# goldbricklemon/uplift-upsample-3dhpe

Hardware: AMD Instinct MI355X
Metric: pose-sequences/sec (higher is better)
Workload: dtype f16x3 (f32 operands split into f16 hi/lo, 3 MFMA passes, f32 accumulate); 1 GPU; config/h36m_351.json forward, N=71 tokens (receptive field 351), J=17, batch 128/GPU, s_in=5, seeded Keras-default weights; global_batch=128, parallelism=batch-sharded x1, hipgraph=True, concurrent_half_batches=False, batches_in_flight=8

## Files before the change

### uplift-upsample-3dhpe_amd/csrc/uu3d_api.hip

```cpp
#include <hip/hip_runtime.h>

#include <algorithm>
#include <cmath>
#include <cstdio>
#include <cstdlib>
#include <cstring>
#include <functional>
#include <map>
#include <mutex>
#include <string>
#include <vector>

#include "../../include/uu3d.h"
#include "uu3d_switches.h"
#include "uu3d_gemm.h"
#include "uu3d_gemm_h3.h"
#include "uu3d_gemm_panel.h"
#include "uu3d_gemm_panel8.h"
#include "uu3d_gemm_wt.h"
#include "uu3d_mlp_fused.h"
#include "uu3d_tchain16.h"
#include "uu3d_attn.h"
#include "uu3d_attn_h3.h"
#include "uu3d_spatial.h"
#include "uu3d_spatial_h3.h"
#include "uu3d_spatial_p16.h"
#include "uu3d_misc.h"
#include "uu3d_metrics.h"
#include "uu3d_tracks.h"
#include "uu3d_stream.h"
#include "uu3d_train.h"
#include "uu3d_bwd.h"
#include "uu3d_launch.h"
#include "uu3d_train_kernels.h"

using namespace uu3d;

namespace {

constexpr int kJ = 17, kDS = 32, kHS = 64, kHeads = 8, kDH = 48;
using SLY2 = SpatialBlockLayoutV2<kDS, kHS>;
constexpr int kFR = 3;
#ifndef UU3D_SPATIAL_MT
#define UU3D_SPATIAL_MT 1
#endif
constexpr int kP16FR = 7, kP16PW = 1;
constexpr int kSpatialMT = UU3D_SPATIAL_MT;

std::string g_create_error;

inline int round_up(int v, int m) { return (v + m - 1) / m * m; }
inline size_t align_up(size_t v, size_t a) { return (v + a - 1) / a * a; }

struct WeightRec {
    std::string name;
    std::vector<int64_t> dims;
    int64_t numel = 0;
    std::vector<float> host;
    bool set = false;
};

struct BlockDev {
    const float *ln1_g, *ln1_b, *wqkv_t, *bqkv, *wp_t, *bp, *ln2_g, *ln2_b, *w1_t, *b1, *w2_t, *b2;
    const float* pe;
    size_t wqkv_pf = 0, w1_pf = 0;
    size_t w2_mf = 0;
    size_t wp_pf = 0;
};

struct ProfRec {
    std::string name, kernel;
    double flops, bytes;
    hipEvent_t e0, e1;
};

}

struct uu3d_train_state;
struct uu3d_model {
    uu3d_config cfg;
    uu3d_train_state* ts = nullptr;
    int device = 0;
    std::vector<WeightRec> weights;
    std::map<std::string, int> index;
    std::vector<int> L;
    Switches sw;
    bool committed = false;
    bool generic = false;
    float* gparams = nullptr;
    float* arena = nullptr;
    size_t arena_floats = 0;
    bool throughput = false;
    struct TcLaunch { int flags; size_t w_off ; size_t p_off ; };
    std::vector<TcLaunch> tchain;
    int num_cus = 256;
    std::recursive_mutex train_mu;
    bool in_commit = false;
    int* d_range = nullptr;
    _Float16* harena = nullptr;
    size_t harena_halfs = 0;
    std::map<size_t, std::pair<size_t, size_t>> hplanes;
    std::map<size_t, size_t> panel_off, mlpf_off;
    SpatialParams sp{};
    size_t sp_frag_off = 0;
// ... 570 lines not shown
```

### uplift-upsample-3dhpe_amd/csrc/uu3d_forward.inc

```

namespace {
struct Workspace {
    float *S, *X, *QKV, *O, *Hb, *XA, *XB, *slab, *mslab;
    unsigned char* tc_scratch;
    int* frame_list;
    float2* stats;
    size_t slab_floats;
    size_t bytes;
};
Workspace carve(const uu3d_model* m, int B, char* base) {
    const uu3d_config& c = m->cfg;
    const size_t rows = (size_t)B * c.num_frames;
    const size_t rows_s = (size_t)B * (c.num_strided > 1 ? std::max(m->L[1], 1) : 1);
    size_t off = 0;
    auto take = [&](size_t n) { size_t o = off; off = align_up(off + n, 256); return o; };
    Workspace w{};
    const size_t oS = take(rows * c.num_keypoints * c.d_spatial * 4);
    const size_t oX = take(rows * c.d_temporal * 4);
    const size_t oQ = take((rows + 128) * 3 * c.d_temporal * 4);
    const size_t oO = take((rows + 32) * c.d_temporal * 4);
    const size_t oH = take((rows + 32) * c.h_temporal * 4);
    const size_t oA = take(rows * c.d_temporal * 4);
    const size_t oB = take(rows_s * c.d_temporal * 4);
    const size_t oT = take(rows * sizeof(float2));
// ... 38 lines not shown
    hipStream_t stream;
    float* slab = nullptr;
    size_t slab_floats = 0;
    bool throughput = false;
    int precision = UU3D_PREC_F16X3;
    int status = UU3D_OK;
    bool few_splits = false;

    void begin(const char* name, const char* kernel, double flops, double bytes) {
        if (!m->profiling) return;
        if (m->prof_used == m->prof.size()) {
            ProfRec r;
            if (hipEventCreate(&r.e0) != hipSuccess || hipEventCreate(&r.e1) != hipSuccess) { status = UU3D_ERR_HIP; return; }
            m->prof.push_back(r);
        }
        ProfRec& r = m->prof[m->prof_used];
        r.name = name; r.kernel = kernel; r.flops = flops; r.bytes = bytes;
        (void)hipEventRecord(r.e0, stream);
    }
    void end() {
        if (m->profiling && m->prof_used < m->prof.size()) { (void)hipEventRecord(m->prof[m->prof_used].e1, stream); ++m->prof_used; }
        hipError_t e = hipGetLastError();
        if (e != hipSuccess && status == UU3D_OK) { status = UU3D_ERR_HIP; m->err = std::string("kernel launch failed: ") + hipGetErrorString(e); }
    }

    template <int BM, int BN, class AL, class EP>
    void gemm_tile(const AL& al, const float* Bt, int M, int N, int Kp, int slices, int kt_per_split, const EP& ep) {
        auto kern = gemm_f32_kernel<BM, BN, AL, EP>;
        constexpr size_t lds = gemm_lds_bytes(BM, BN);
        allow_lds<gemm_f32_kernel<BM, BN, AL, EP>>(lds);
        const int mt = (M + BM - 1) / BM, nt = (N + BN - 1) / BN;
        const int grid = round_up(mt, 8) * nt;
        hipLaunchKernelGGL(kern, dim3(grid, slices), dim3(256), lds, stream, al, Bt, M, N, Kp, mt, nt, kt_per_split, ep);
    }

    template <int TM, int TN, class AL, class EP>
    void gemm_h3_tile(const AL& al, const _Float16* Bh, const _Float16* Bl, int M, int N, int Kp, int slices, int kt_per_split, const EP& ep) {
        auto kern = gemm_h3_kernel<TM, TN, AL, EP>;
        auto kern_deep = gemm_h3_kernel<TM, TN, AL, EP, 1>;
        constexpr size_t lds = gemm_h3_lds_bytes(64 * TM, 64 * TN);
        allow_lds<gemm_h3_kernel<TM, TN, AL, EP>>(lds); allow_lds<gemm_h3_kernel<TM, TN, AL, EP, 1>>(lds);
        const int mt = (M + 64 * TM - 1) / (64 * TM), nt = (N + 64 * TN - 1) / (64 * TN);
        const int grid = round_up(mt, 8) * nt;
        if (gemm_h3_deep(grid * slices)) hipLaunchKernelGGL(kern_deep, dim3(grid, slices), dim3(256), lds, stream, al, Bh, Bl, M, N, Kp, mt, nt, kt_per_split, ep);
        else hipLaunchKernelGGL(kern, dim3(grid, slices), dim3(256), lds, stream, al, Bh, Bl, M, N, Kp, mt, nt, kt_per_split, ep);
    }

    template <int TM, int TN, class GL, class EP>
    void gemm_h3g_tile(const GL& gl, const _Float16* Bh, const _Float16* Bl, int M, int N, int Kp, int slices, int kt_per_split, const EP& ep) {
        auto kern = gemm_h3g_kernel<TM, TN, GL, EP>;
        constexpr size_t lds = gemm_h3g_lds_bytes(64 * TM, 64 * TN);
        allow_lds<gemm_h3g_kernel<TM, TN, GL, EP>>(lds);
        const int mt = (M + 64 * TM - 1) / (64 * TM), nt = (N + 64 * TN - 1) / (64 * TN);
        const int grid = round_up(mt, 8) * nt;
        hipLaunchKernelGGL(kern, dim3(grid, slices), dim3(256), lds, stream, gl, Bh, Bl, M, N, Kp, mt, nt, kt_per_split, ep);
    }

    int splitk_target() const {
        return (throughput && few_splits) ? process_switches().thr_splitk_target : 768;
    }
    template <class GL, class EP>
    void gemm_g(const char* name, const GL& gl, const float* Bt, int M, int N, int K, const EP& ep, double extra_bytes = 0) {
        const int KT = K / 32;
        const int tiles = ((M + 63) / 64) * ((N + 63) / 64);
        const auto [slices, kps] = splitk_rule(M, N, KT, splitk_target(), slab_floats, true);
        const int ldslab = round_up(N, 4);
        begin(name, "gemm_h3", 2.0 * M * (double)N * K, 4.0 * ((double)M * K + (double)N * K + (double)M * N) + extra_bytes);
        const auto it = m->hplanes.find((size_t)(Bt - m->arena));
        if ((K % 32) != 0 || it == m->hplanes.end()) { status = UU3D_ERR_INVALID_ARGUMENT; m->err = "gemm_g: operand without f16 planes or K % 32 != 0"; end(); return; }
        const _Float16* Bh = m->harena + it->second.first; const _Float16* Bl = m->harena + it->second.second;
        if (slices == 1) {
            if (N % 128 == 0 && tiles >= 256) gemm_h3g_tile<1, 2>(gl, Bh, Bl, M, N, K, 1, KT, ep);
            else gemm_h3g_tile<1, 1>(gl, Bh, Bl, M, N, K, 1, KT, ep);
        } else {
            EpSlab es{slab, ldslab, (size_t)M * ldslab};
            if (N % 128 == 0 && tiles >= 200) gemm_h3g_tile<1, 2>(gl, Bh, Bl, M, N, K, slices, kps, es);
            else gemm_h3g_tile<1, 1>(gl, Bh, Bl, M, N, K, slices, kps, es);
            hipLaunchKernelGGL(splitk_reduce_kernel<EP>, dim3((M * N + 255) / 256), dim3(256), 0, stream,
                               slab, slices, (size_t)M * ldslab, M, N, ldslab, ep);
        }
        end();
    }

    static int panel_splits(int M, int N) {
        const int mt = (M + 127) / 128, chunks = N / 32;
        int best = 0; double best_cost = 1e30;
        for (int S = 1; S <= chunks; ++S) {
            if (chunks % S != 0 || chunks / S > PANEL_COLV_FLOATS / 32) continue;
            const int per_xcd = (mt * S + 7) / 8;
            const double cost = (double)((per_xcd + 31) / 32) * (2.5 + (double)chunks / S);
            if (cost < best_cost) { best_cost = cost; best = S; }
        }
        return best;
    }
    bool panel_ok(int M, int N, int K, size_t pf) const {
        return !m->sw.no_panel && pf != 0 && K == 384 && N % 32 == 0 && M >= 1024 && (double)M * N * 4.0 < 4.0e9;
    }
    static bool panel8_ok(int cpw) {
        return !process_switches().panel4 && (cpw == 4 || cpw == 6 || cpw == 8 || cpw == 9 || cpw == 12);
    }
    template <class EP> static const char* panel_symbol(bool eight) {
        const char* e = std::is_same<EP, PanelEpBiasSplitQ>::value ? "BiasSplitQ" : std::is_same<EP, PanelEpBiasResidual>::value ? "BiasResidual"
                      : std::is_same<EP, PanelEpBiasResidualLn>::value ? "BiasResidualLn" : std::is_same<EP, PanelEpBiasReluSplit>::value ? "BiasReluSplit"
                      : std::is_same<EP, PanelEpBiasRelu>::value ? "BiasRelu" : "Bias";
        static thread_local char buf[32];
        std::snprintf(buf, sizeof buf, "%s<%s>", eight ? "gemm_panel8" : "gemm_panel", e);
        return buf;
    }
    template <class EP>
    bool launch_panel8(const _Float16* Af, const _Float16* Bf, const float* colv, int M, int mt, int S, int cpw, const EP& ep) {
        if (!panel8_ok(cpw)) return false;
        const dim3 grid(8 * S, ((mt * S + 7) / 8 + S - 1) / S);
#define UU3D_P8_LAUNCH(CPW) { allow_lds<gemm_h3_panel8_kernel<EP, CPW, 3>>(P8_LDS_TOTAL); \
            hipLaunchKernelGGL((gemm_h3_panel8_kernel<EP, CPW, 3>), grid, dim3(512), P8_LDS_TOTAL, stream, Af, Bf, colv, M, mt, S, ep); return true; }
        switch (cpw) {
            case 4: UU3D_P8_LAUNCH(4)
            case 6: UU3D_P8_LAUNCH(6)
            case 8: UU3D_P8_LAUNCH(8)
            case 9: UU3D_P8_LAUNCH(9)
            case 12: UU3D_P8_LAUNCH(12)
            default: return false;
        }
#undef UU3D_P8_LAUNCH
    }
    template <class EP, int CPW = 0>
    void launch_panel4(const _Float16* Af, const _Float16* Bf, const float* colv, int M, int mt, int S, int cpw, const EP& ep) {
        allow_lds<gemm_h3_panel_kernel<24, EP, CPW>>(PANEL_LDS_TOTAL);
        hipLaunchKernelGGL((gemm_h3_panel_kernel<24, EP, CPW>), dim3(8 * S, ((mt * S + 7) / 8 + S - 1) / S), dim3(256), PANEL_LDS_TOTAL, stream, Af, Bf, colv, M, mt, S, cpw, ep);
    }
    template <class EP>
    void gemm_panel_at(const char* name, const _Float16* Af, const _Float16* Bf, const float* colv, int M, int N, const EP& ep, int S = 0) {
        const int K = 384, mt = (M + 127) / 128;
        if (S == 0) S = panel_splits(M, N);
        begin(name, panel_symbol<EP>(panel8_ok((N / 32) / S)), 2.0 * M * (double)N * K, 4.0 * ((double)M * K + (double)N * K + (double)M * N));
        if (!launch_panel8(Af, Bf, colv, M, mt, S, (N / 32) / S, ep)) launch_panel4(Af, Bf, colv, M, mt, S, (N / 32) / S, ep);
        end();
    }
    template <class EP>
    void gemm_panel(const char* name, const _Float16* Af, size_t pf, const float* colv, int M, int N, const EP& ep) {
        if (skip_mask() & 2) return;
        const int s = process_switches().panel_s;
        gemm_panel_at(name, Af, m->harena + pf, colv, M, N, ep, (s != 0 && (N / 32) % s == 0 && (N / 32) / s <= PANEL_COLV_FLOATS / 32) ? s : 0);
    }
    bool gemm_panel_residual(const char* name, const _Float16* Af, size_t pf, const float* colv, int M, float* x,
                             const float* ln_g = nullptr, const float* ln_b = nullptr, _Float16* ln_out = nullptr) {
        const int K = 384, N = 384, mt = (M + 127) / 128;
        if (skip_mask() & 4) return false;
        int S = 1; double best = 1e30;
        for (int s : {1, 2, 3}) {
            const int per_xcd = (mt * s + 7) / 8;
            const double cost = (double)((per_xcd + 31) / 32) * (2.5 + 12.0 / s);
            if (cost < best) { best = cost; S = s; }
        }
        if (throughput && mt >= 64) S = 1;
        if (process_switches().panel_proj_s != 0) S = process_switches().panel_proj_s;
        const bool ln_tail = S == 1 && ln_out != nullptr && !process_switches().no_ln_tail && panel8_ok(12);
        begin(name, ln_tail ? panel_symbol<PanelEpBiasResidualLn>(true) : panel_symbol<PanelEpBiasResidual>(panel8_ok(12 / S)),
              2.0 * M * (double)N * K, 4.0 * ((double)M * K + (double)N * K + 2.0 * (double)M * N));
        const PanelEpBiasResidual ep{x, N};
        if (ln_tail) {
            const PanelEpBiasResidualLn epl{{x, N}, ln_g, ln_b, 1e-5f, ln_out};
            if (launch_panel8(Af, m->harena + pf, colv, M, mt, 1, 12, epl)) { end(); return true; }
        }
        if (launch_panel8(Af, m->harena + pf, colv, M, mt, S, 12 / S, ep)) { end(); return false; }
        if (S == 3) launch_panel4<PanelEpBiasResidual, 4>(Af, m->harena + pf, colv, M, mt, S, 4, ep);
        else if (S == 2) launch_panel4<PanelEpBiasResidual, 6>(Af, m->harena + pf, colv, M, mt, S, 6, ep);
// ... 160 lines not shown
            UU3D_ATTN_CASE(5) UU3D_ATTN_CASE(6) UU3D_ATTN_CASE(7) UU3D_ATTN_CASE(8)
            default: status = UU3D_ERR_UNSUPPORTED; m->err = "attention over more than 128 tokens needs the f16x3 path (precision f16x3, d_t and h_t multiples of 32)"; break;
        }
#undef UU3D_ATTN_CASE
        end();
    }
};

template <class EP>
void spatial_stage(Launcher& Lh, const uu3d_config& c, const float* kp2d, int M, const uint8_t* mask, int* frame_list, float* S, bool timing_skip, const EP& ep) {
    uu3d_model* const m = Lh.m;
    const int J = c.num_keypoints, ds = c.d_spatial, dt = c.d_temporal;
    const bool h3 = c.precision == UU3D_PREC_F16X3 && !m->sw.spatial_f32 && (m->sw.spatial_h3_always || spatial_h3_pays(M));
    const bool planes = h3 && !m->sw.no_planes && (J * ds) % 32 == 0;
    const bool skip = timing_skip && (skip_mask() & 1);
    SpatialParams sp = m->sp;
    sp.total_frames = M;
    sp.frame_list = nullptr;
    if (mask != nullptr) {
        Lh.begin("compact_frames", "compact_frames", 0.0, (double)M * 5.0);
        hipLaunchKernelGGL(compact_frames_kernel, dim3(1), dim3(1024), 0, Lh.stream, mask, M, frame_list);
        Lh.end();
        sp.frame_list = frame_list;
    }
    const double fl = (double)M * (2.0 * J * 2 * ds + c.spatial_depth * (4.0 * 2 * J * ds * ds + 8.0 * 4 * J * J * (ds / 8) + 2.0 * 2 * J * ds * kHS));
    _Float16* const s_hi = planes ? reinterpret_cast<_Float16*>(S) : (_Float16*)nullptr;
    _Float16* const s_lo = planes ? reinterpret_cast<_Float16*>(S) + (size_t)M * J * ds : (_Float16*)nullptr;
    if (h3 && m->sw.spatial_h3_tiles) {
        Lh.begin("spatial_stack", "spatial_h3", fl, 4.0 * M * J * (2.0 + ds));
        if (!skip)
        hipLaunchKernelGGL((spatial_stack_h3_kernel<kJ, kFR, kSpatialMT>), dim3((M + kFR - 1) / kFR), dim3(64 * (2 / kSpatialMT)), sh3::lds_bytes(), Lh.stream, kp2d, sp,
                           m->harena + m->sp_frag_off, S, s_hi, s_lo, SpatialTrainIO{});
        Lh.end();
    } else if (h3) {
        Lh.begin("spatial_stack", "spatial_p16", fl, 4.0 * M * J * (2.0 + ds));
        if (!skip)
        hipLaunchKernelGGL((spatial_stack_p16_kernel<kJ, kP16FR, kP16PW>), dim3((M + kP16FR - 1) / kP16FR), dim3(64 * p16_waves(kJ, kP16FR, kP16PW)), sp16::lds_bytes<kP16FR>(c.spatial_depth),
                           Lh.stream, kp2d, sp, m->harena + m->sp_frag16_off, S, s_hi, s_lo);
        Lh.end();
    } else {
        Lh.begin("spatial_stack", "spatial_mfma", fl, 4.0 * M * J * (2.0 + ds));
        hipLaunchKernelGGL((spatial_stack_mfma_kernel<kJ, kFR>), dim3((M + kFR - 1) / kFR), dim3(64), spatial_v2_lds_bytes(), Lh.stream, kp2d, sp, S);
        Lh.end();
    }
    if (planes) Lh.gemm_g("s2t", GLoadPlain{s_hi, s_lo, J * ds, M}, m->s2t_wt, M, dt, J * ds, ep);
    else Lh.gemm("s2t", ALoadPlain{S, J * ds, M, J * ds}, m->s2t_wt, M, dt, J * ds, ep);
}

}

int uu3d_forward(uu3d_model* m, const float* kp2d, const uint8_t* mask, int32_t B, float* full_out,
                 float* central_out, void* workspace, size_t workspace_bytes, void* stream_) {
    return uu3d_forward_attention(m, kp2d, mask, B, full_out, central_out, nullptr, workspace, workspace_bytes, stream_);
}

int uu3d_forward_attention(uu3d_model* m, const float* kp2d, const uint8_t* mask, int32_t B, float* full_out,
                           float* central_out, float* const* attn_out, void* workspace, size_t workspace_bytes, void* stream_) {
    if (!m) return UU3D_ERR_INVALID_ARGUMENT;
    return uu3d_forward_ex(m, kp2d, mask, B, full_out, central_out, attn_out, workspace, workspace_bytes,
                           m->throughput ? UU3D_SCHEDULE_THROUGHPUT : UU3D_SCHEDULE_LATENCY, stream_);
}

namespace {
struct FramesIn { const float* features; long num_rows; const int32_t* rows; };

constexpr int kFewRows = 512;

struct Forward {
    uu3d_model* const m;
    Launcher Lh;
    const Workspace w;
    const uu3d_config c;
    const uint8_t* const mask;
    const int B;
    float* const full_out; float* const central_out; float* const* const attn_out;
    const bool part_body, part_tail;

    const int N = c.num_frames, J = c.num_keypoints, dt = c.d_temporal, ht = c.h_temporal, M = B * N;
    const bool has_h1 = c.full_output && c.temporal_depth > 0;
    const bool planes = (c.precision == UU3D_PREC_F16X3) && (dt % 32 == 0) && (ht % 32 == 0) && !m->sw.no_planes;
    const bool chain = Lh.throughput && planes && m->sw.tchain_mode != 0 && (m->sw.tchain_mode == 1 || (M + 127) / 128 >= m->sw.tchain_min_tiles) && !m->tchain.empty() && M >= 1024 &&
                       (Lh.attn_is_h3(N, true) || (m->sw.tchain_short && Lh.attn_h3_any(N))) && (c.num_strided == 0 || m->L[0] == N) && (double)M * 1152 * 4.0 < 4.0e9 &&
                       attn_out == nullptr;
    _Float16* const Ph = reinterpret_cast<_Float16*>(w.O);
    _Float16* const Hh = reinterpret_cast<_Float16*>(w.Hb);
    const BlockDev* pend = nullptr;
    float* xa = w.XA;
    char nm[48];

    void tokens_from_frames(const FramesIn& frames) {
        Lh.begin("frames_to_tokens", "frames_to_tokens", 0.0, 4.0 * 3.0 * M * dt);
        hipLaunchKernelGGL(frames_to_tokens_kernel, dim3((unsigned)(((size_t)M * (dt / 4) + 255) / 256)), dim3(256), 0, Lh.stream,
                           frames.features, frames.num_rows, frames.rows, mask, m->token, m->pe_t, (long)M, N, dt, w.X);
        Lh.end();
    }
    void spatial(const float* kp2d) {
        spatial_stage(Lh, c, kp2d, M, mask, w.frame_list, w.S, true, EpSpatialToTemporal{w.X, m->s2t_b, dt, mask, m->token, m->pe_t, N});
    }

    const _Float16* block_head(const char* tag, int i, const BlockDev& b, float* x, int L, const uint8_t* kmask, const BlockDev* prev, bool fuse_mlp) {
        const int Mr = B * L;
        auto name = [&](const char* what) { snprintf(nm, sizeof nm, "%s%d.%s", tag, i + 1, what); return nm; };
        _Float16* const Pl = Ph + (size_t)Mr * dt; _Float16* const Hl = Hh + (size_t)Mr * ht;
        const bool qsplit = Lh.attn_is_h3(L, planes);
        _Float16* const Qh = reinterpret_cast<_Float16*>(w.QKV); _Float16* const Ql = Qh + (size_t)Mr * 3 * dt;
        const EpBiasSplitQ ep_qs{Qh, Ql, b.bqkv, 3 * dt, dt, Lh.attn_qscale()};
        const bool few = planes && Mr <= kFewRows && Lh.wt_ok(b.wqkv_t, dt) && Lh.wt_ok(b.w1_t, dt);
        auto maps = [&]() {
            if (attn_out != nullptr && tag[0] == 't' && attn_out[i] != nullptr) {
                Lh.begin(name("attn_maps"), "attn_probs", 2.0 * B * (double)c.num_heads * L * L * kDH, 4.0 * B * (double)c.num_heads * L * L);
                const size_t lds = (size_t)L * (kDH + 1) * sizeof(float);
                allow_lds<attn_probs_kernel>(160 * 1024 - 256);
                if (qsplit) hipLaunchKernelGGL(attn_probs_kernel, dim3(B * c.num_heads), dim3(256), lds, Lh.stream, (const void*)Qh, (const _Float16*)Ql, 3 * dt, dt, L, c.num_heads, kDH, kmask, 1.0f, 1, attn_out[i]);
                else hipLaunchKernelGGL(attn_probs_kernel, dim3(B * c.num_heads), dim3(256), lds, Lh.stream, (const void*)w.QKV, (const _Float16*)nullptr, 3 * dt, dt, L, c.num_heads, kDH, kmask, 1.0f / sqrtf((float)kDH), 0, attn_out[i]);
                Lh.end();
            }
        };
        if (few) {
            WtLoadF32 l1{x, dt, Mr, dt, b.ln1_g, b.ln1_b, 1e-5f, 1};
            if (qsplit) Lh.gemm_wt(name("ln_qkv"), l1, b.wqkv_t, Mr, 3 * dt, dt, ep_qs);
            else Lh.gemm_wt(name("ln_qkv"), l1, b.wqkv_t, Mr, 3 * dt, dt, EpBias{w.QKV, b.bqkv, 3 * dt});
            maps();
            Lh.attn(name("attn"), w.QKV, B, L, kmask, w.O, (size_t)Mr * dt);
            { GLoadPlain gl{Ph, Pl, dt, Mr}; Lh.gemm_g(name("proj_res"), gl, b.wp_t, Mr, dt, dt, EpBiasResidual{x, b.bp, dt, nullptr, nullptr, 1}, 4.0 * Mr * dt); }
            WtLoadF32 l2{x, dt, Mr, dt, b.ln2_g, b.ln2_b, 1e-5f, 1};
            Lh.gemm_wt(name("ln_fc1"), l2, b.w1_t, Mr, ht, dt, EpBiasReluSplit{Hh, Hl, b.b1, ht});
            return nullptr;
        }
        if (prev != nullptr) {
            if (x == w.X) Lh.ln_res_split_frag(name("ln1_split"), w.X, Mr, prev->b2, w.mslab, nullptr, nullptr, 1, b.ln1_g, b.ln1_b, Ph);
            else Lh.ln_res_split_frag(name("ln1_split"), w.X, Mr, prev->b2, w.mslab, x, b.pe, L, b.ln1_g, b.ln1_b, Ph);
            if (qsplit) Lh.gemm_panel(name("ln_qkv"), Ph, b.wqkv_pf, b.bqkv, Mr, 3 * dt, PanelEpBiasSplitQ{Qh, Ql, 3 * dt, dt, Lh.attn_qscale()});
            else Lh.gemm_panel(name("ln_qkv"), Ph, b.wqkv_pf, b.bqkv, Mr, 3 * dt, PanelEpBias{w.QKV, 3 * dt});
        } else if (planes && Lh.panel_ok(Mr, 3 * dt, dt, b.wqkv_pf)) {
            Lh.ln_split_frag(name("ln1_split"), x, Mr, b.ln1_g, b.ln1_b, Ph);
            if (qsplit) Lh.gemm_panel(name("ln_qkv"), Ph, b.wqkv_pf, b.bqkv, Mr, 3 * dt, PanelEpBiasSplitQ{Qh, Ql, 3 * dt, dt, Lh.attn_qscale()});
            else Lh.gemm_panel(name("ln_qkv"), Ph, b.wqkv_pf, b.bqkv, Mr, 3 * dt, PanelEpBias{w.QKV, 3 * dt});
        } else {
            Lh.row_stats(name("stats1"), x, dt, Mr, w.stats);
            ALoadLayerNorm al{x, w.stats, b.ln1_g, b.ln1_b, dt, Mr, dt};
            if (qsplit) Lh.gemm(name("ln_qkv"), al, b.wqkv_t, Mr, 3 * dt, dt, ep_qs);
            else { EpBias ep{w.QKV, b.bqkv, 3 * dt}; Lh.gemm(name("ln_qkv"), al, b.wqkv_t, Mr, 3 * dt, dt, ep); }
        }
        maps();
        const bool pproj = planes && !m->sw.no_panel_proj && Lh.panel_ok(Mr, dt, dt, b.wp_pf);
        Lh.attn(name("attn"), w.QKV, B, L, kmask, w.O, planes ? (size_t)Mr * dt : 0, pproj);
        const bool mlp_panel = planes && Lh.panel_ok(Mr, ht, dt, b.w1_pf);
        bool ln2_done = false;
        if (pproj) ln2_done = mlp_panel ? Lh.gemm_panel_residual(name("proj_res"), Ph, b.wp_pf, b.bp, Mr, x, b.ln2_g, b.ln2_b, Ph)
                                        : Lh.gemm_panel_residual(name("proj_res"), Ph, b.wp_pf, b.bp, Mr, x);
        else {
            EpBiasResidual ep{x, b.bp, dt, nullptr, nullptr, 1};
            if (planes) { GLoadPlain gl{Ph, Pl, dt, Mr}; Lh.gemm_g(name("proj_res"), gl, b.wp_t, Mr, dt, dt, ep, 4.0 * Mr * dt); }
            else { ALoadPlain al{w.O, dt, Mr, dt}; Lh.gemm(name("proj_res"), al, b.wp_t, Mr, dt, dt, ep, 4.0 * Mr * dt); }
        }
        if (mlp_panel) {
            if (!ln2_done) Lh.ln_split_frag(name("ln2_split"), x, Mr, b.ln2_g, b.ln2_b, Ph);
            if (fuse_mlp) return Ph;
            Lh.gemm_panel(name("ln_fc1"), Ph, b.w1_pf, b.b1, Mr, ht, PanelEpBiasReluSplit{Hh, Hl, ht});
        } else {
            Lh.row_stats(name("stats2"), x, dt, Mr, w.stats);
            ALoadLayerNorm al{x, w.stats, b.ln2_g, b.ln2_b, dt, Mr, dt};
            if (planes) { EpBiasReluSplit ep{Hh, Hl, b.b1, ht}; Lh.gemm(name("ln_fc1"), al, b.w1_t, Mr, ht, dt, ep); }
            else { EpBiasRelu ep{w.Hb, b.b1, ht}; Lh.gemm(name("ln_fc1"), al, b.w1_t, Mr, ht, dt, ep); }
        }
        return nullptr;
    }

    void temporal_chain() {
        _Float16* const Q = reinterpret_cast<_Float16*>(w.QKV);
        Lh.tchain("t1.ln_qkv", m->tchain[0], M, nullptr, w.X, nullptr, nullptr, 1, Q, nullptr, w.tc_scratch);
        for (int i = 0; i < c.temporal_depth; ++i) {
            const bool masked = c.has_strided_input && i < c.first_strided_token_attention_layer;
            snprintf(nm, sizeof nm, "t%d.attn", i + 1);
            Lh.attn(nm, w.QKV, B, N, masked ? mask : nullptr, w.O, (size_t)M * dt, true, true);
            const bool to_strided = i + 1 == c.temporal_depth && c.num_strided > 0;
            snprintf(nm, sizeof nm, "t%d.chain", i + 1);
            Lh.tchain(nm, m->tchain[i + 1], M, Ph, w.X, to_strided ? w.XA : nullptr, to_strided ? m->sblocks[0].pe : nullptr, N, Q, nullptr, w.tc_scratch);
        }
    }
    void temporal_blocks() {
        for (int i = 0; i < c.temporal_depth; ++i) {
            const BlockDev& b = m->tblocks[i];
            const bool masked = c.has_strided_input && i < c.first_strided_token_attention_layer;
            const bool last = (i + 1 == c.temporal_depth);
            const bool fuse = planes && Lh.mlpf_ok(M, b) && (last ? (c.num_strided > 0 && Lh.panel_ok(M, 3 * dt, dt, m->sblocks[0].wqkv_pf))
                                                                  : Lh.panel_ok(M, 3 * dt, dt, m->tblocks[i + 1].wqkv_pf));
            const _Float16* const a2 = block_head("t", i, b, w.X, N, masked ? mask : nullptr, pend, fuse);
            pend = nullptr;
            if (fuse) {
                snprintf(nm, sizeof nm, "t%d.mlp", i + 1);
                Lh.mlp_fused(nm, a2, b, M, w.mslab);
                pend = &b;
                continue;
            }
            const bool to_strided = last && c.num_strided > 0;
            EpBiasResidual ep_fc2{w.X, b.b2, dt, to_strided ? w.XA : nullptr, to_strided ? m->sblocks[0].pe : nullptr, N};
            snprintf(nm, sizeof nm, "t%d.fc2_res", i + 1);
            if (planes) { GLoadPlain gl{Hh, Hh + (size_t)M * ht, ht, M}; Lh.gemm_g(nm, gl, b.w2_t, M, dt, ht, ep_fc2, 4.0 * M * dt); }
            else { ALoadPlain al{w.Hb, ht, M, ht}; Lh.gemm(nm, al, b.w2_t, M, dt, ht, ep_fc2, 4.0 * M * dt); }
        }
    }
    void head1() {
        if (!has_h1) return;
        ALoadPlain al{w.X, dt, M, dt}; EpBias ep{full_out, m->h1_b, 3 * J};
        Lh.gemm("head1", al, m->h1_wt, M, 3 * J, dt, ep);
    }
    void strided_blocks() {
        float* xb = w.XB;
        const _Float16* const hzero = m->harena;
        if (c.temporal_depth == 0 && c.num_strided > 0) {
            Lh.begin("s1.add_pe", "add_pe", 0.0, 12.0 * M * dt);
            hipLaunchKernelGGL(add_period_kernel, dim3((unsigned)(((size_t)M * dt / 4 + 255) / 256)), dim3(256), 0, Lh.stream, w.X, m->sblocks[0].pe, M, dt, N, w.XA);
            Lh.end();
        }
        for (int i = 0; i < c.num_strided; ++i) {
            const BlockDev& b = m->sblocks[i];
            const int Li = m->L[i], Lo = m->L[i + 1], Mi = B * Li, Mo = B * Lo;
            if (((skip_mask() & 256) || part_body) && i >= 1) continue;
            if (((skip_mask() & 512) || part_tail) && i == 0) { std::swap(xa, xb); xb = w.XA; continue; }
            const int lo = (c.strides[i] > 1 && c.pad_left[i] == 0) ? 1 : 0;
            const EpConvResidual ep_conv{xb, b.b2, dt, xa, Li, Lo, c.strides[i], lo,
                                         (i + 1 < c.num_strided) ? m->sblocks[i + 1].pe : nullptr};
            const bool smask = c.temporal_depth == 0 && c.has_strided_input && i < c.first_strided_token_attention_layer;
            if (chain && i == 0) {
                Lh.attn("s1.attn", w.QKV, B, Li, nullptr, w.O, (size_t)Mi * dt, true, true);
                Lh.tchain("s1.chain", m->tchain[c.temporal_depth + 1], Mi, Ph, nullptr, xa, nullptr, 1, nullptr, Hh, w.tc_scratch);
            } else
            block_head("s", i, b, xa, Li, smask ? mask : nullptr, i == 0 ? pend : nullptr, false);
            if (i == 0) head1();
            snprintf(nm, sizeof nm, "s%d.conv_res", i + 1);
            if (planes) { GLoadConv3 gl{Hh, Hh + (size_t)Mi * ht, hzero, ht, Li, Lo, c.strides[i], c.pad_left[i], Mo};
                          Lh.gemm_g(nm, gl, b.w2_t, Mo, dt, 3 * ht, ep_conv, 4.0 * Mo * dt); }
            else { ALoadConv3 al{w.Hb, ht, Li, Lo, c.strides[i], c.pad_left[i], Mo, 3 * ht};
                   Lh.gemm(nm, al, b.w2_t, Mo, dt, 3 * ht, ep_conv, 4.0 * Mo * dt); }
            std::swap(xa, xb);
            if (i == 0) xb = w.XA;
        }
    }
    void head2() {
        ALoadPlain al{c.num_strided > 0 ? xa : w.X + (size_t)(N / 2) * dt, c.num_strided > 0 ? dt : N * dt, B, dt};
        EpBias ep{central_out, m->h2_b, 3 * J};
        Lh.gemm("head2", al, m->h2_wt, B, 3 * J, dt, ep);
    }
    void range_check() {
        if (c.precision != UU3D_PREC_F16X3) return;
        Lh.begin("range_check", "range_check", 0.0, 4.0 * ((has_h1 ? (double)M * 3 * J : 0.0) + (double)B * 3 * J));
        hipLaunchKernelGGL(range_check_kernel, dim3(256), dim3(256), 0, Lh.stream, has_h1 ? full_out : central_out, has_h1 ? (long)M * 3 * J : 0L,
                           central_out, (long)B * 3 * J, m->d_range);
        Lh.end();
    }
};

int forward_impl(uu3d_model* m, const float* kp2d, const FramesIn* frames, const uint8_t* mask, int32_t B, float* full_out,
                 float* central_out, float* const* attn_out, void* workspace, size_t workspace_bytes, int32_t schedule, void* stream_) {
    if (!m) return UU3D_ERR_INVALID_ARGUMENT;
    const bool exact_f32 = (schedule & UU3D_SCHEDULE_EXACT_F32) != 0;
    schedule &= ~UU3D_SCHEDULE_EXACT_F32;
#ifdef UU3D_TIMING_BUILD
    const bool parts_ok = process_switches().timing_parts;
#else
    constexpr bool parts_ok = false;
#endif
    const bool part_body = parts_ok && (schedule & 0x200) != 0, part_tail = parts_ok && (schedule & 0x400) != 0;
    if (parts_ok) schedule &= ~0x600;
    if (schedule != UU3D_SCHEDULE_LATENCY && schedule != UU3D_SCHEDULE_THROUGHPUT) return fail(m, UU3D_ERR_INVALID_ARGUMENT, "schedule must be UU3D_SCHEDULE_LATENCY or UU3D_SCHEDULE_THROUGHPUT");
    if (!m->committed) return fail(m, UU3D_ERR_NOT_READY, "uu3d_commit_weights has not been called");
    if ((!kp2d && !frames) || !central_out || !workspace || B < 1) return fail(m, UU3D_ERR_INVALID_ARGUMENT, "null buffer or batch < 1");
    if (frames != nullptr) {
        if (m->generic) return fail(m, UU3D_ERR_UNSUPPORTED, "uu3d_forward_frames_ex: handles with generic dims have no frames form (compiled dims only)");
        if (!frames->features || !frames->rows || frames->num_rows < 1) return fail(m, UU3D_ERR_INVALID_ARGUMENT, "uu3d_forward_frames_ex: null features / rows or no feature rows");
        if (((uintptr_t)frames->features & 15) != 0 || (m->cfg.d_temporal % 4) != 0) return fail(m, UU3D_ERR_INVALID_ARGUMENT, "uu3d_forward_frames_ex: features must be 16-byte aligned");
    }
    uu3d_config c = m->cfg;
    if (exact_f32) {
        if (m->generic) return fail(m, UU3D_ERR_UNSUPPORTED, "UU3D_SCHEDULE_EXACT_F32: handles with generic dims have no exact-f32 forward");
        if (c.num_frames > 128) return fail(m, UU3D_ERR_UNSUPPORTED, "UU3D_SCHEDULE_EXACT_F32: the exact-f32 attention holds sequences of <= 128 tokens");
        c.precision = UU3D_PREC_F32;
    }
    if ((c.has_strided_input != 0) != (mask != nullptr))
        return fail(m, UU3D_ERR_INVALID_ARGUMENT, "stride_mask must be given iff the model has strided input");
    if (c.full_output && c.temporal_depth > 0 && !full_out) return fail(m, UU3D_ERR_INVALID_ARGUMENT, "full_out_dev is required for this model");
    if (((uintptr_t)workspace & 255) != 0) return fail(m, UU3D_ERR_WORKSPACE, "workspace must be 256-byte aligned");
    if (m->generic) {
        const int r = generic_forward(m, kp2d, mask, B, full_out, central_out, attn_out, workspace, workspace_bytes, stream_);
        if (r == UU3D_OK && c.precision == UU3D_PREC_F16X3) {
            const bool has_full = c.full_output && c.temporal_depth > 0 && full_out != nullptr;
            hipLaunchKernelGGL(range_check_kernel, dim3(256), dim3(256), 0, (hipStream_t)stream_, has_full ? full_out : central_out,
                               has_full ? (long)B * c.num_frames * c.num_keypoints * 3 : 0L, central_out, (long)B * c.num_keypoints * 3, m->d_range);
        }
        return r;
    }
    const Workspace w = carve(m, B, (char*)workspace);
    if (workspace_bytes < w.bytes) return fail(m, UU3D_ERR_WORKSPACE, "workspace smaller than uu3d_workspace_bytes(batch)");
    if ((long)B * c.num_frames * c.num_keypoints > (1L << 30)) return fail(m, UU3D_ERR_INVALID_ARGUMENT, "batch too large");

    HIPCHK(m, hipSetDevice(m->device));
    m->prof_used = 0;
    Forward f{m, Launcher{m, (hipStream_t)stream_, w.slab, w.slab_floats, schedule == UU3D_SCHEDULE_THROUGHPUT, c.precision}, w, c,
              mask, B, full_out, central_out, attn_out, part_body, part_tail};
    if (!part_tail) { if (frames != nullptr) f.tokens_from_frames(*frames); else f.spatial(kp2d); }
    f.Lh.few_splits = f.chain;
    if (!part_tail) {
        if (f.chain) f.temporal_chain(); else f.temporal_blocks();
        if (c.num_strided == 0) f.head1();
    }
    f.strided_blocks();
    if (!part_body) { f.head2(); f.range_check(); }
    return f.Lh.status;
}
}


int uu3d_forward_ex(uu3d_model* m, const float* kp2d, const uint8_t* mask, int32_t B, float* full_out,
                    float* central_out, float* const* attn_out, void* workspace, size_t workspace_bytes, int32_t schedule, void* stream_) {
    return forward_impl(m, kp2d, nullptr, mask, B, full_out, central_out, attn_out, workspace, workspace_bytes, schedule, stream_);
}

int uu3d_forward_frames_ex(uu3d_model* m, const float* features, int64_t num_rows, const int32_t* rows, const uint8_t* mask, int32_t B,
                           float* full_out, float* central_out, float* const* attn_out, void* workspace, size_t workspace_bytes,
                           int32_t schedule, void* stream_) {
    if (!m) return UU3D_ERR_INVALID_ARGUMENT;
    const FramesIn fin{features, (long)num_rows, rows};
    return forward_impl(m, nullptr, &fin, mask, B, full_out, central_out, attn_out, workspace, workspace_bytes, schedule, stream_);
}

namespace {
struct FrameWorkspace { float *S, *slab; size_t slab_floats, bytes; };
FrameWorkspace carve_frames(const uu3d_model* m, long F, char* base) {
// ... 46 lines not shown
```

### uplift-upsample-3dhpe_amd/csrc/uu3d_switches.h

```cpp
#pragma once
#include <cstdio>
#include <cstdlib>
#include <string>

namespace uu3d {

struct Switches {
    bool spatial_f32 = false;
    bool spatial_h3_always = false;
    bool spatial_h3_tiles = false;
    bool no_planes = false;
    bool attn_wg = false;
    bool no_mlpf = false;
    bool no_wt = false;
    bool attn_f32 = false;
    bool no_panel = false;
    bool no_panel_proj = false;
    int tchain_mode = -1;
    int tchain_min_tiles = 8;
    bool tchain_short = true;
    struct Train {
        bool f32 = false;
        bool one_stream = false;
        bool event_flags_set = false;
        unsigned event_flags = 0;
        bool any_queue = false;
        bool spatial_unfused = false;
        bool no_panel = false;
        bool attn_bwd_generic = false;
    } train;
};

inline Switches read_switches() {
    Switches s;
    auto is1 = [](const char* name) { const char* e = getenv(name); return e != nullptr && e[0] == '1'; };
    auto present = [](const char* name) { return getenv(name) != nullptr; };
    { const char* e = getenv("UU3D_SPATIAL"); const std::string v = e ? e : "";
      s.spatial_f32 = v == "f32"; s.spatial_h3_always = v == "h3"; s.spatial_h3_tiles = v == "h3tiles"; }
    s.no_planes = is1("UU3D_NO_PLANES");
    s.attn_wg = is1("UU3D_ATTN_WG");
    s.no_mlpf = is1("UU3D_NO_MLPF");
    s.no_wt = is1("UU3D_NO_WT");
    s.attn_f32 = is1("UU3D_ATTN_F32");
    s.no_panel = is1("UU3D_NO_PANEL");
    s.no_panel_proj = is1("UU3D_NO_PANEL_PROJ");
    { const char* e = getenv("UU3D_TCHAIN"); if (e != nullptr && (e[0] == '0' || e[0] == '1')) s.tchain_mode = e[0] - '0'; }
    { const char* e = getenv("UU3D_TCHAIN_MIN_TILES"); if (e != nullptr && atoi(e) > 0) s.tchain_min_tiles = atoi(e); }
    { const char* e = getenv("UU3D_TCHAIN_SHORT"); if (e != nullptr) s.tchain_short = atoi(e) != 0; }
    s.train.f32 = present("UU3D_TRAIN_F32");
    s.train.one_stream = present("UU3D_TRAIN_1STREAM");
    { const char* e = getenv("UU3D_TRAIN_EVENT_FLAGS"); s.train.event_flags_set = e != nullptr; if (e) s.train.event_flags = (unsigned)strtoul(e, nullptr, 0); }
    s.train.any_queue = present("UU3D_TRAIN_ANY_QUEUE");
    s.train.spatial_unfused = present("UU3D_TRAIN_SPATIAL_UNFUSED");
    s.train.no_panel = present("UU3D_TRAIN_NO_PANEL");
    s.train.attn_bwd_generic = present("UU3D_ATTN_BWD_GENERIC");
    return s;
}

struct ProcessSwitches {
#ifdef UU3D_TIMING_BUILD
    int skip = 0;
    bool timing_parts = false;
#endif
    bool panel4 = false;
    int panel_s = 0;
    int panel_proj_s = 0;
    bool no_ln_tail = false;
    int thr_splitk_target = 192;
    int tnh_wgs = 192;
    int gemm_deep_wgs = 640;
    bool tn_f32 = false;
    bool capture_inorder = false;
};

inline const ProcessSwitches& process_switches() {
    static const ProcessSwitches sw = [] {
        ProcessSwitches s;
#ifdef UU3D_TIMING_BUILD
        { const char* e = getenv("UU3D_SKIP"); s.skip = e ? atoi(e) : 0;
          if (s.skip) fprintf(stderr, "[uu3d] UU3D_SKIP=%d: launches are being skipped, RESULTS ARE WRONG (timing experiment)\n", s.skip); }
        { const char* e = getenv("UU3D_TIMING_PARTS"); s.timing_parts = e != nullptr && atoi(e) != 0; }
#endif
        { const char* e = getenv("UU3D_PANEL4"); s.panel4 = e != nullptr && atoi(e) != 0; }
        { const char* e = getenv("UU3D_PANEL_S"); if (e != nullptr && e[0] >= '1' && e[0] <= '3') s.panel_s = e[0] - '0'; }
        { const char* e = getenv("UU3D_PANEL_PROJ_S"); if (e != nullptr && e[0] >= '1' && e[0] <= '3') s.panel_proj_s = e[0] - '0'; }
        s.no_ln_tail = getenv("UU3D_NO_LN_TAIL") != nullptr;
        { const char* e = getenv("UU3D_THR_SPLITK_TARGET"); if (e != nullptr && atoi(e) > 0) s.thr_splitk_target = atoi(e); }
        { const char* e = getenv("UU3D_TNH_WGS"); if (e != nullptr) s.tnh_wgs = atoi(e); }
        { const char* e = getenv("UU3D_GEMM_DEEP_WGS"); if (e != nullptr) s.gemm_deep_wgs = atoi(e); }
        s.tn_f32 = getenv("UU3D_TN_F32") != nullptr;
        s.capture_inorder = getenv("UU3D_TRAIN_CAPTURE_INORDER") != nullptr;
        return s;
    }();
    return sw;
}

}
```

Measured before the change: 219,200 pose-sequences/s.

## Fuse last strided conv split-K reduce, residual, head2 and range check into tail kernel

When the final strided block reduces to one token, the last conv GEMM now writes its split-K partials to slabs. A new tail kernel sums the slabs, adds the conv bias and the residual, runs the head2 projection and flags non-finite outputs in a single launch. The non-finite check is also folded into the head1 epilogue, so the separate split-K reduce, head2 GEMM and range_check launches are dropped. The cost is an extra hand-written kernel whose head2 weights sit in registers, plus atomics on the range flag.

Result: no change. 218,300 pose-sequences/s (-0.4%).

```diff
diff --git a/uplift-upsample-3dhpe_amd/csrc/uu3d_api.hip b/uplift-upsample-3dhpe_amd/csrc/uu3d_api.hip
--- a/uplift-upsample-3dhpe_amd/csrc/uu3d_api.hip
+++ b/uplift-upsample-3dhpe_amd/csrc/uu3d_api.hip
@@ -20,6 +20,7 @@
 #include "uu3d_gemm_wt.h"
 #include "uu3d_mlp_fused.h"
 #include "uu3d_tchain16.h"
+#include "uu3d_tail.h"
 #include "uu3d_attn.h"
 #include "uu3d_attn_h3.h"
 #include "uu3d_spatial.h"
diff --git a/uplift-upsample-3dhpe_amd/csrc/uu3d_forward.inc b/uplift-upsample-3dhpe_amd/csrc/uu3d_forward.inc
--- a/uplift-upsample-3dhpe_amd/csrc/uu3d_forward.inc
+++ b/uplift-upsample-3dhpe_amd/csrc/uu3d_forward.inc
@@ -144,6 +144,25 @@
         end();
     }
 
+    template <class GL>
+    int gemm_g_slabs(const char* name, const GL& gl, const float* Bt, int M, int N, int K, double extra_bytes = 0) {
+        const int KT = K / 32;
+        const int tiles = ((M + 63) / 64) * ((N + 63) / 64);
+        const auto [slices, kps] = splitk_rule(M, N, KT, splitk_target(), slab_floats, true);
+        const int ldslab = round_up(N, 4);
+        begin(name, "gemm_h3", 2.0 * M * (double)N * K, 4.0 * ((double)M * K + (double)N * K + (double)M * N) + extra_bytes);
+        const auto it = m->hplanes.find((size_t)(Bt - m->arena));
+        if ((K % 32) != 0 || it == m->hplanes.end() || (size_t)slices * M * ldslab > slab_floats) {
+            status = UU3D_ERR_INVALID_ARGUMENT; m->err = "gemm_g_slabs: operand without f16 planes, K % 32 != 0 or slab too small"; end(); return 0;
+        }
+        const _Float16* Bh = m->harena + it->second.first; const _Float16* Bl = m->harena + it->second.second;
+        EpSlab es{slab, ldslab, (size_t)M * ldslab};
+        if (N % 128 == 0 && tiles >= 200) gemm_h3g_tile<1, 2>(gl, Bh, Bl, M, N, K, slices, kps, es);
+        else gemm_h3g_tile<1, 1>(gl, Bh, Bl, M, N, K, slices, kps, es);
+        end();
+        return slices;
+    }
+
     static int panel_splits(int M, int N) {
         const int mt = (M + 127) / 128, chunks = N / 32;
         int best = 0; double best_cost = 1e30;
@@ -470,6 +489,9 @@
     const bool chain = Lh.throughput && planes && m->sw.tchain_mode != 0 && (m->sw.tchain_mode == 1 || (M + 127) / 128 >= m->sw.tchain_min_tiles) && !m->tchain.empty() && M >= 1024 &&
                        (Lh.attn_is_h3(N, true) || (m->sw.tchain_short && Lh.attn_h3_any(N))) && (c.num_strided == 0 || m->L[0] == N) && (double)M * 1152 * 4.0 < 4.0e9 &&
                        attn_out == nullptr;
+    const bool tail = chain && !m->sw.no_tail && c.num_strided > 0 && m->L[c.num_strided] == 1 && dt == TAIL_D && 3 * J <= TAIL_WAVES * TAIL_NJ &&
+                      (size_t)B * dt <= w.slab_floats;
+    bool tail_done = false;
     _Float16* const Ph = reinterpret_cast<_Float16*>(w.O);
     _Float16* const Hh = reinterpret_cast<_Float16*>(w.Hb);
     const BlockDev* pend = nullptr;
@@ -591,8 +613,9 @@
     }
     void head1() {
         if (!has_h1) return;
-        ALoadPlain al{w.X, dt, M, dt}; EpBias ep{full_out, m->h1_b, 3 * J};
-        Lh.gemm("head1", al, m->h1_wt, M, 3 * J, dt, ep);
+        ALoadPlain al{w.X, dt, M, dt};
+        if (tail) Lh.gemm("head1", al, m->h1_wt, M, 3 * J, dt, EpBiasRange{full_out, m->h1_b, 3 * J, m->d_range});
+        else Lh.gemm("head1", al, m->h1_wt, M, 3 * J, dt, EpBias{full_out, m->h1_b, 3 * J});
     }
     void strided_blocks() {
         float* xb = w.XB;
@@ -618,6 +641,18 @@
             block_head("s", i, b, xa, Li, smask ? mask : nullptr, i == 0 ? pend : nullptr, false);
             if (i == 0) head1();
             snprintf(nm, sizeof nm, "s%d.conv_res", i + 1);
+            if (tail && i + 1 == c.num_strided) {
+                GLoadConv3 gl{Hh, Hh + (size_t)Mi * ht, hzero, ht, Li, Lo, c.strides[i], c.pad_left[i], Mo};
+                const int slices = Lh.gemm_g_slabs(nm, gl, b.w2_t, Mo, dt, 3 * ht, 4.0 * Mo * dt);
+                if (slices < 1) return;
+                snprintf(nm, sizeof nm, "s%d.tail", i + 1);
+                Lh.begin(nm, "tail", 2.0 * B * 3.0 * J * dt, 4.0 * ((double)slices * B * dt + (double)B * dt + 3.0 * J * dt + 3.0 * J * B));
+                const TailArgs ta{w.slab, slices, (size_t)Mo * dt, dt, b.b2, xa, Li, lo, m->h2_wt, m->h2_b, B, 3 * J, central_out, m->d_range};
+                hipLaunchKernelGGL(tail_head2_kernel, dim3((B + TAIL_ROWS - 1) / TAIL_ROWS), dim3(64 * TAIL_WAVES), 0, Lh.stream, ta);
+                Lh.end();
+                tail_done = true;
+                return;
+            }
             if (planes) { GLoadConv3 gl{Hh, Hh + (size_t)Mi * ht, hzero, ht, Li, Lo, c.strides[i], c.pad_left[i], Mo};
                           Lh.gemm_g(nm, gl, b.w2_t, Mo, dt, 3 * ht, ep_conv, 4.0 * Mo * dt); }
             else { ALoadConv3 al{w.Hb, ht, Li, Lo, c.strides[i], c.pad_left[i], Mo, 3 * ht};
@@ -627,12 +662,13 @@
         }
     }
     void head2() {
+        if (tail_done) return;
         ALoadPlain al{c.num_strided > 0 ? xa : w.X + (size_t)(N / 2) * dt, c.num_strided > 0 ? dt : N * dt, B, dt};
         EpBias ep{central_out, m->h2_b, 3 * J};
         Lh.gemm("head2", al, m->h2_wt, B, 3 * J, dt, ep);
     }
     void range_check() {
-        if (c.precision != UU3D_PREC_F16X3) return;
+        if (c.precision != UU3D_PREC_F16X3 || tail_done) return;
         Lh.begin("range_check", "range_check", 0.0, 4.0 * ((has_h1 ? (double)M * 3 * J : 0.0) + (double)B * 3 * J));
         hipLaunchKernelGGL(range_check_kernel, dim3(256), dim3(256), 0, Lh.stream, has_h1 ? full_out : central_out, has_h1 ? (long)M * 3 * J : 0L,
                            central_out, (long)B * 3 * J, m->d_range);
diff --git a/uplift-upsample-3dhpe_amd/csrc/uu3d_switches.h b/uplift-upsample-3dhpe_amd/csrc/uu3d_switches.h
--- a/uplift-upsample-3dhpe_amd/csrc/uu3d_switches.h
+++ b/uplift-upsample-3dhpe_amd/csrc/uu3d_switches.h
@@ -19,6 +19,7 @@
     int tchain_mode = -1;
     int tchain_min_tiles = 8;
     bool tchain_short = true;
+    bool no_tail = false;
     struct Train {
         bool f32 = false;
         bool one_stream = false;
@@ -47,6 +48,7 @@
     { const char* e = getenv("UU3D_TCHAIN"); if (e != nullptr && (e[0] == '0' || e[0] == '1')) s.tchain_mode = e[0] - '0'; }
     { const char* e = getenv("UU3D_TCHAIN_MIN_TILES"); if (e != nullptr && atoi(e) > 0) s.tchain_min_tiles = atoi(e); }
     { const char* e = getenv("UU3D_TCHAIN_SHORT"); if (e != nullptr) s.tchain_short = atoi(e) != 0; }
+    { const char* e = getenv("UU3D_TAIL"); s.no_tail = e != nullptr && e[0] == '0'; }
     s.train.f32 = present("UU3D_TRAIN_F32");
     s.train.one_stream = present("UU3D_TRAIN_1STREAM");
     { const char* e = getenv("UU3D_TRAIN_EVENT_FLAGS"); s.train.event_flags_set = e != nullptr; if (e) s.train.event_flags = (unsigned)strtoul(e, nullptr, 0); }
diff --git a/uplift-upsample-3dhpe_amd/csrc/uu3d_tail.h b/uplift-upsample-3dhpe_amd/csrc/uu3d_tail.h
--- /dev/null
+++ b/uplift-upsample-3dhpe_amd/csrc/uu3d_tail.h
@@ -0,0 +1,96 @@
+#pragma once
+#include <hip/hip_runtime.h>
+#include <cstddef>
+
+namespace uu3d {
+
+constexpr int TAIL_D = 384;
+constexpr int TAIL_ROWS = 2;
+constexpr int TAIL_WAVES = 4;
+constexpr int TAIL_NJ = 16;
+
+struct EpBiasRange {
+    float* __restrict__ out; const float* __restrict__ bias; int ldo; int* __restrict__ flag;
+    __device__ __forceinline__ float2 colv(int col) const { return make_float2(bias[col], 0.f); }
+    __device__ __forceinline__ float2 pre(int, int) const { return make_float2(0.f, 0.f); }
+    __device__ __forceinline__ void store(int row, int col, float v, float2 cv, float2) const {
+        const float y = v + cv.x;
+        out[(size_t)row * ldo + col] = y;
+        if (!(fabsf(y) <= 3.0e38f)) atomicOr(flag, 1);
+    }
+};
+
+struct TailArgs {
+    const float* slab; int slices; size_t slice_stride; int ldslab;
+    const float* conv_bias;
+    const float* xin; int L_in, lo;
+    const float* Wt; const float* hbias;
+    int B, N;
+    float* out;
+    int* flag;
+};
+
+static __global__ void __launch_bounds__(64 * TAIL_WAVES)
+tail_head2_kernel(const TailArgs a)
+{
+    __shared__ float y[TAIL_ROWS][TAIL_D];
+    const int lane = threadIdx.x & 63, wave = threadIdx.x >> 6;
+    const int b0 = blockIdx.x * TAIL_ROWS;
+
+    float2 w[TAIL_NJ][3];
+#pragma unroll
+    for (int q = 0; q < TAIL_NJ; ++q) {
+        const int j = min(wave + TAIL_WAVES * q, a.N - 1);
+        const float* wr = a.Wt + (size_t)j * TAIL_D + 2 * lane;
+#pragma unroll
+        for (int i = 0; i < 3; ++i) w[q][i] = *reinterpret_cast<const float2*>(wr + 128 * i);
+    }
+
+    for (int e = threadIdx.x; e < TAIL_ROWS * TAIL_D; e += 64 * TAIL_WAVES) {
+        const int r = e / TAIL_D, c = e - r * TAIL_D;
+        const int b = min(b0 + r, a.B - 1);
+        const float* p = a.slab + (size_t)b * a.ldslab + c;
+        const float id = a.xin[((size_t)b * a.L_in + a.lo) * TAIL_D + c];
+        const float cb = a.conv_bias[c];
+        float v = p[0];
+        int s = 1;
+        for (; s + 7 < a.slices; s += 8) {
+            float t[8];
+#pragma unroll
+            for (int u = 0; u < 8; ++u) t[u] = p[(size_t)(s + u) * a.slice_stride];
+#pragma unroll
+            for (int u = 0; u < 8; ++u) v += t[u];
+        }
+        for (; s + 1 < a.slices; s += 2) { const float t0 = p[(size_t)s * a.slice_stride], t1 = p[(size_t)(s + 1) * a.slice_stride]; v += t0; v += t1; }
+        if (s < a.slices) v += p[(size_t)s * a.slice_stride];
+        y[r][c] = id + (v + cb);
+    }
+    __syncthreads();
+
+    float2 x[TAIL_ROWS][3];
+#pragma unroll
+    for (int r = 0; r < TAIL_ROWS; ++r)
+#pragma unroll
+        for (int i = 0; i < 3; ++i) x[r][i] = *reinterpret_cast<const float2*>(&y[r][2 * lane + 128 * i]);
+#pragma unroll
+    for (int q = 0; q < TAIL_NJ; ++q) {
+        const int j = wave + TAIL_WAVES * q;
+        if (j >= a.N) break;
+        const float hb = a.hbias[j];
+#pragma unroll
+        for (int r = 0; r < TAIL_ROWS; ++r) {
+            float acc = 0.f;
+#pragma unroll
+            for (int i = 0; i < 3; ++i) { acc = fmaf(x[r][i].x, w[q][i].x, acc); acc = fmaf(x[r][i].y, w[q][i].y, acc); }
+#pragma unroll
+            for (int d = 32; d >= 1; d >>= 1) acc += __shfl_xor(acc, d, 64);
+            if (lane == 0 && b0 + r < a.B) {
+                const float o = acc + hb;
+                a.out[(size_t)(b0 + r) * a.N + j] = o;
+                if (!(fabsf(o) <= 3.0e38f)) atomicOr(a.flag, 1);
+            }
+        }
+    }
+}
+
+}
```
